# amazon-science/gnn-tail-generalization

Hardware: AMD Instinct MI355X
Metric: teachergnn_fullgraph_train_steps_per_sec (higher is better)
Workload: dtype f32

## Files before the change

### gnn-tail-generalization_amd/csrc/cb_front.hip

```cpp
#include "cb_common.h"
#include "cb_limb_core.h"
#include "cb_philox.h"
#include "cb_tile_gemm.h"

namespace cb {

struct FrontArgs {
  const float* x;
  int64_t ld_x;
  const uint4* image_in;
  const float* bias_in;
  const uint4* image_0;
  const float* rowscale;
  const float* addend;
  int64_t ld_add;
  float* x0;
  int64_t ld_x0;
  unsigned long long* bits;
  float* x0_drop;
  int64_t ld_drop;
  float* z0;
  int64_t ld_z;
  int64_t M;
  uint32_t thresh;
  float keep_scale;
  uint64_t seed_x, seed_x0;
  const uint64_t* seed_dev;
  int64_t row0;
  int n_tiles;
};

template <int NS1>
__global__ void __launch_bounds__(256, 2) k_front(FrontArgs fa) {
  constexpr int K1 = 16 * NS1, LDX = K1 + 4, NV = kTM * K1 / 4 / 256;
  static_assert(NV >= 1 && kTM * LDX <= kTM * kTLD, "x tile must fit the region of the X0 tile");
  __shared__ __attribute__((aligned(16))) float tile[kTM * kTLD];
  constexpr int kScratch = 2 * RowOperand<kTM>::BYTES > 4 * 8 * kCLD * 4 ? 2 * RowOperand<kTM>::BYTES : 4 * 8 * kCLD * 4;
  __shared__ __attribute__((aligned(16))) char scratch[kScratch];
  float (*cstrip)[8 * kCLD] = reinterpret_cast<float (*)[8 * kCLD]>(scratch);
  __shared__ float rs_tile[2][kTM];
  const int t = threadIdx.x, lane = t & 63, w = __builtin_amdgcn_readfirstlane(t >> 6);
  const uint64_t sx = fa.seed_dev ? fa.seed_x + *fa.seed_dev : fa.seed_x, s0 = fa.seed_dev ? fa.seed_x0 + *fa.seed_dev : fa.seed_x0;
  float4 xr[NV];
  auto load_x = [&](int tile_id) {
    const int64_t m0 = (int64_t)tile_id * kTM;
#pragma unroll
    for (int j = 0; j < NV; ++j) {
      const int idx = t + 256 * j, row = idx / (K1 / 4), c4 = idx % (K1 / 4);
      const int64_t m = m0 + row;
      xr[j] = (tile_id < fa.n_tiles && m < fa.M) ? *reinterpret_cast<const float4*>(fa.x + m * fa.ld_x + 4 * c4) : make_float4(0.f, 0.f, 0.f, 0.f);
    }
  };
  float bvec[4] = {0.f, 0.f, 0.f, 0.f};
  if (fa.bias_in) {
#pragma unroll
    for (int i = 0; i < 4; ++i) bvec[i] = fa.bias_in[4 * lane + i];
  }
  int par = 0;
  for (int tile_id = blockIdx.x; tile_id < fa.n_tiles; tile_id += gridDim.x, par ^= 1) {
    const int64_t m0 = (int64_t)tile_id * kTM;
    load_x(tile_id);
#pragma unroll
    for (int j = 0; j < NV; ++j) {
      const int idx = t + 256 * j, row = idx / (K1 / 4), c4 = idx % (K1 / 4);
      float v[4] = {xr[j].x, xr[j].y, xr[j].z, xr[j].w};
      if (fa.thresh) {
        float mk[4];
        keep4(sx, ((fa.row0 + m0 + row) * K1 + 4 * c4) >> 2, fa.thresh, fa.keep_scale, mk);
#pragma unroll
        for (int i = 0; i < 4; ++i) v[i] = mul_rounded(v[i], mk[i]);
      }
      *reinterpret_cast<float4*>(tile + row * LDX + 4 * c4) = make_float4(v[0], v[1], v[2], v[3]);
    }
    if (t < kTM) rs_tile[par][t] = (fa.rowscale && m0 + t < fa.M) ? fa.rowscale[m0 + t] : 1.f;
    __syncthreads();
    f32x16 acc[2][2];
    tile_times_image_coop<NS1, LDX, 1>(tile, scratch, fa.image_in, w, lane, t, acc);
    {
      const int l31 = lane & 31, lh = lane >> 5;
#pragma unroll
      for (int i = 0; i < 2; ++i)
#pragma unroll
        for (int j = 0; j < 2; ++j)
#pragma unroll
          for (int reg = 0; reg < 16; ++reg)
            tile[(32 * i + (reg & 3) + 8 * (reg >> 2) + 4 * lh) * kTLD + 64 * w + 32 * j + l31] = acc[i][j][reg];
    }
    __syncthreads();
#pragma unroll 4
    for (int r = 0; r < 16; ++r) {
      const int row = 16 * w + r;
      const int64_t m = m0 + row;
      float* tp = tile + row * kTLD + 4 * lane;
      const float4 v = *reinterpret_cast<const float4*>(tp);
      float o[4] = {v.x, v.y, v.z, v.w};
#pragma unroll
      for (int i = 0; i < 4; ++i) o[i] = fmaxf(o[i] + bvec[i], 0.f);
      float xd[4] = {o[0], o[1], o[2], o[3]};
      if (fa.thresh) {
        float mk[4];
        keep4(s0, ((fa.row0 + m) * kND + 4 * lane) >> 2, fa.thresh, fa.keep_scale, mk);
#pragma unroll
        for (int i = 0; i < 4; ++i) xd[i] = o[i] * mk[i];
      }
      *reinterpret_cast<float4*>(tp) = make_float4(xd[0], xd[1], xd[2], xd[3]);
      if (m < fa.M) {
        store_stream4(fa.x0 + m * fa.ld_x0 + 4 * lane, o);
        if (fa.bits) {
          unsigned long long mine = 0ull;
#pragma unroll
          for (int k = 0; k < 4; ++k) {
            const unsigned long long wq = __ballot(o[k] > 0.f);
            if (lane == k) mine = wq;
          }
          if (lane < 4) fa.bits[m * 4 + lane] = mine;
        }
        if (fa.x0_drop) store_stream4(fa.x0_drop + m * fa.ld_drop + 4 * lane, xd);
      }
    }
    __syncthreads();
    tile_times_image_coop<kNS, kTLD, 1>(tile, scratch, fa.image_0, w, lane, t, acc);
    acc_rows_through_strip(acc, cstrip[w], w, lane, [&](int row, int n, const float4& v) {
      const int64_t m = m0 + row;
      if (m < fa.M) {
        const float rs = rs_tile[par][row];
        float ad[4] = {0.f, 0.f, 0.f, 0.f};
        if (fa.addend) {
          const float4 a4 = *reinterpret_cast<const float4*>(fa.addend + m * fa.ld_add + n);
          ad[0] = a4.x; ad[1] = a4.y; ad[2] = a4.z; ad[3] = a4.w;
        }
        const float zero_bias = 0.f;
        float o[4] = {v.x, v.y, v.z, v.w};
#pragma unroll
        for (int e = 0; e < 4; ++e) o[e] = o[e] * rs + ad[e] + zero_bias;
        store_stream4(fa.z0 + m * fa.ld_z + n, o);
      }
    });
  }
}

static inline bool fr_al16(const void* p) { return ((uintptr_t)p % 16) == 0; }

}

using namespace cb;

extern "C" size_t cb_front_image_bytes(int64_t K) {
  if (K != 64 && K != 128) return 0;
  return (size_t)(K / 16) * kNT * 3 * 64 * sizeof(uint4);
}

extern "C" int cb_front_image_f32(const float* W, int64_t ld, int64_t K, int transpose, void* image, size_t image_bytes, void* stream) {
  CB_CHECK_ARG(cb_front_image_bytes(K) > 0, CB_E_INVALID, "cb_front_image_f32: K must be 64 or 128 (got %lld)", (long long)K);
  CB_CHECK_ARG(W && image && ld >= (transpose ? K : kND), CB_E_INVALID, "cb_front_image_f32: null pointer / bad leading dimension");
  CB_CHECK_ARG(image_bytes >= cb_front_image_bytes(K) && fr_al16(image), CB_E_WORKSPACE, "cb_front_image_f32: image buffer too small or misaligned");
  const int64_t sk = transpose ? 1 : ld, sn = transpose ? ld : 1;
  const int ns = (int)(K / 16);
  hipLaunchKernelGGL(k_weight_image, dim3(ns * kNT * 64 / 256), dim3(256), 0, (hipStream_t)stream, W, sk, sn, (uint4*)image, ns);
  CB_LAUNCH_CHECK();
  return CB_OK;
}

extern "C" int cb_trunk_front_f32(const float* x, int64_t ld_x, int64_t M, int64_t K, const void* image_in, const float* bias_in, const void* image_0,
                                  const float* rowscale, const float* addend, int64_t ld_add, float* x0, int64_t ld_x0, uint64_t* relu_bits,
                                  float* x0_drop, int64_t ld_drop, float* z0, int64_t ld_z, float drop_p, uint64_t seed_x, uint64_t seed_x0,
                                  const uint64_t* seed_dev, int64_t row0, void* stream) {
  CB_CHECK_ARG(M >= 0 && cb_front_image_bytes(K) > 0 && drop_p >= 0.f && drop_p < 1.f && row0 >= 0, CB_E_INVALID,
               "cb_trunk_front_f32: bad size (K must be 64 or 128; hidden width 256) or p");
  CB_CHECK_ARG(M < ((int64_t)1 << 31) * kTM / 2, CB_E_RANGE, "cb_trunk_front_f32: size out of range");
  if (M == 0) return CB_OK;
  CB_CHECK_ARG(x && image_in && image_0 && x0 && z0, CB_E_INVALID, "cb_trunk_front_f32: null pointer");
  CB_CHECK_ARG(fr_al16(x) && ld_x % 4 == 0 && ld_x >= K && fr_al16(image_in) && fr_al16(image_0) && fr_al16(x0) && ld_x0 % 4 == 0 && ld_x0 >= kND &&
                   fr_al16(z0) && ld_z % 4 == 0 && ld_z >= kND && (!addend || (fr_al16(addend) && ld_add % 4 == 0 && ld_add >= kND)) &&
                   (!x0_drop || (fr_al16(x0_drop) && ld_drop % 4 == 0 && ld_drop >= kND)) && (!relu_bits || (uintptr_t)relu_bits % 8 == 0),
               CB_E_INVALID, "cb_trunk_front_f32: 16-byte aligned rows required");
  FrontArgs fa{x, ld_x, (const uint4*)image_in, bias_in, (const uint4*)image_0, rowscale, addend, ld_add, x0, ld_x0, (unsigned long long*)relu_bits,
               x0_drop, ld_drop, z0, ld_z, M};
  fa.thresh = drop_p > 0.f ? dropout_threshold(drop_p) : 0u;
  fa.keep_scale = 1.f / (1.f - drop_p);
  fa.seed_x = seed_x; fa.seed_x0 = seed_x0; fa.seed_dev = seed_dev; fa.row0 = row0;
  fa.n_tiles = (int)((M + kTM - 1) / kTM);
  int dev = 0, n_cu = 0;
  if (hipGetDevice(&dev) != hipSuccess || hipDeviceGetAttribute(&n_cu, hipDeviceAttributeMultiprocessorCount, dev) != hipSuccess || n_cu <= 0) n_cu = 256;
  const int blocks = fa.n_tiles < 2 * n_cu ? fa.n_tiles : 2 * n_cu;
  const dim3 grid((unsigned)blocks), blk(256);
  hipStream_t st = (hipStream_t)stream;
  if (K == 64) hipLaunchKernelGGL((k_front<4>), grid, blk, 0, st, fa);
  else hipLaunchKernelGGL((k_front<8>), grid, blk, 0, st, fa);
  CB_LAUNCH_CHECK();
  return CB_OK;
}
```

### gnn-tail-generalization_amd/csrc/cb_tile_gemm.h

```cpp
#pragma once
#include "cb_common.h"
#include "cb_limb_core.h"

namespace cb {

constexpr int kTM = 64;
constexpr int kTLD = 260;
constexpr int kKD = 256;
constexpr int kND = 256;
constexpr int kNT = kND / 32, kNS = kKD / 16;

__global__ void __launch_bounds__(256) k_weight_image(const float* __restrict__ W, int64_t sk, int64_t sn, uint4* __restrict__ image, int n_steps);

__device__ __forceinline__ bf16x8 as_bf16x8(const uint4& v) { return __builtin_bit_cast(bf16x8, v); }

__device__ __forceinline__ void store_stream4(float* __restrict__ p, const float (&v)[4]) {
  typedef float f4_t __attribute__((ext_vector_type(4)));
  const f4_t q = {v[0], v[1], v[2], v[3]};
  __builtin_nontemporal_store(q, reinterpret_cast<f4_t*>(p));
}

template <int NSTEPS, int TLD, int PF = 1>
__device__ __forceinline__ void tile_times_image(const float* __restrict__ tile, const uint4* __restrict__ image, int w, int lane, f32x16 (&acc)[2][2]) {
  static_assert(PF >= 1 && PF <= 3 && PF < NSTEPS, "prefetch distance");
  const int l31 = lane & 31, lh = lane >> 5;
#pragma unroll
  for (int i = 0; i < 2; ++i)
#pragma unroll
    for (int j = 0; j < 2; ++j)
#pragma unroll
      for (int e = 0; e < 16; ++e) acc[i][j][e] = 0.f;
  const float* a_row[2] = {tile + l31 * TLD + 8 * lh, tile + (32 + l31) * TLD + 8 * lh};
  const uint4* bp = image + ((int64_t)(2 * w) * 3) * 64 + lane;
  uint4 bq[PF + 1][2][3];
#pragma unroll
  for (int d = 0; d < PF; ++d) {
#pragma unroll
    for (int j = 0; j < 2; ++j)
#pragma unroll
      for (int p = 0; p < 3; ++p) bq[d][j][p] = bp[j * 192 + p * 64];
    bp += kNT * 192;
  }
  auto step = [&](int s, int cur, int nx) {
    if (s + PF < NSTEPS) {
#pragma unroll
      for (int j = 0; j < 2; ++j)
#pragma unroll
        for (int p = 0; p < 3; ++p) bq[nx][j][p] = bp[j * 192 + p * 64];
    }
    bp += kNT * 192;
#pragma unroll
    for (int i = 0; i < 2; ++i) {
      const float4 x0 = *reinterpret_cast<const float4*>(a_row[i] + 16 * s);
      const float4 x1 = *reinterpret_cast<const float4*>(a_row[i] + 16 * s + 4);
      uint32_t hh[4], mm[4], ll[4];
      split3x2(x0.x, x0.y, hh[0], mm[0], ll[0]);
      split3x2(x0.z, x0.w, hh[1], mm[1], ll[1]);
      split3x2(x1.x, x1.y, hh[2], mm[2], ll[2]);
      split3x2(x1.z, x1.w, hh[3], mm[3], ll[3]);
      const bf16x8 a_hi = as_bf16x8(make_uint4(hh[0], hh[1], hh[2], hh[3]));
      const bf16x8 a_mid = as_bf16x8(make_uint4(mm[0], mm[1], mm[2], mm[3]));
      const bf16x8 a_lo = as_bf16x8(make_uint4(ll[0], ll[1], ll[2], ll[3]));
#define CB_TG_MFMA2(A_, P_) \
  _Pragma("unroll") for (int j = 0; j < 2; ++j) acc[i][j] = __builtin_amdgcn_mfma_f32_32x32x16_bf16(A_, as_bf16x8(bq[cur][j][P_]), acc[i][j], 0, 0, 0);
      CB_TG_MFMA2(a_lo, 0)
      CB_TG_MFMA2(a_hi, 2)
      CB_TG_MFMA2(a_mid, 1)
      CB_TG_MFMA2(a_mid, 0)
      CB_TG_MFMA2(a_hi, 1)
      CB_TG_MFMA2(a_hi, 0)
#undef CB_TG_MFMA2
    }
  };
  constexpr int R = PF + 1, MAIN = NSTEPS / R * R;
#pragma unroll 1
  for (int s0 = 0; s0 < MAIN; s0 += R) {
#pragma unroll
    for (int r = 0; r < R; ++r) step(s0 + r, r, (r + PF) % R);
  }
#pragma unroll
  for (int r = 0; r < NSTEPS - MAIN; ++r) step(MAIN + r, r, (r + PF) % R);
}

template <int NSTEPS, int TLD, int PF = 1>
__device__ __forceinline__ void tile_times_image_coop(const float* __restrict__ tile, char* __restrict__ planes, const uint4* __restrict__ image, int w, int lane,
                                                      int t, f32x16 (&acc)[2][2]) {
  using OA = RowOperand<kTM>;
  static_assert(OA::NV == 1 && PF >= 1 && PF <= 3 && PF < NSTEPS, "64-row tiles, one float4 of the slab per thread");
#pragma unroll
  for (int i = 0; i < 2; ++i)
#pragma unroll
    for (int j = 0; j < 2; ++j)
#pragma unroll
      for (int e = 0; e < 16; ++e) acc[i][j][e] = 0.f;
  const int row = t >> 2, kq = t & 3;
  const float* a_src = tile + row * TLD + 4 * kq;
  const uint32_t woff = row * 32 + (((kq >> 1) ^ ((row >> 3) & 1)) << 4) + ((kq & 1) << 3);
  const uint32_t aaddr[2] = {OA::frag_addr(0, lane), OA::frag_addr(32, lane)};
  auto stage = [&](int s, char* dst) {
    const float4 x = *reinterpret_cast<const float4*>(a_src + 16 * s);
    const float v[4] = {x.x, x.y, x.z, x.w};
    uint2 pl[3];
    split4(v, pl);
#pragma unroll
    for (int p = 0; p < 3; ++p) *reinterpret_cast<uint2*>(dst + p * OA::PLANE + woff) = pl[p];
  };
  const uint4* bp = image + ((int64_t)(2 * w) * 3) * 64 + lane;
  uint4 bq[PF + 1][2][3];
#pragma unroll
  for (int d = 0; d < PF; ++d) {
#pragma unroll
    for (int j = 0; j < 2; ++j)
#pragma unroll
      for (int p = 0; p < 3; ++p) bq[d][j][p] = bp[j * 192 + p * 64];
    bp += kNT * 192;
  }
  stage(0, planes);
  __syncthreads();
  auto step = [&](int s, int cur, int nx) {
    if (s + PF < NSTEPS) {
#pragma unroll
      for (int j = 0; j < 2; ++j)
#pragma unroll
        for (int p = 0; p < 3; ++p) bq[nx][j][p] = bp[j * 192 + p * 64];
    }
    bp += kNT * 192;
    const char* S = planes + (s & 1) * OA::BYTES;
    if (s + 1 < NSTEPS) stage(s + 1, planes + ((s + 1) & 1) * OA::BYTES);
#pragma unroll
    for (int i = 0; i < 2; ++i) {
      const bf16x8 a_lo = OA::frag(S, aaddr[i], 2), a_hi = OA::frag(S, aaddr[i], 0), a_mid = OA::frag(S, aaddr[i], 1);
#define CB_TG_MFMA2(A_, P_) \
  _Pragma("unroll") for (int j = 0; j < 2; ++j) acc[i][j] = __builtin_amdgcn_mfma_f32_32x32x16_bf16(A_, as_bf16x8(bq[cur][j][P_]), acc[i][j], 0, 0, 0);
      CB_TG_MFMA2(a_lo, 0)
      CB_TG_MFMA2(a_hi, 2)
      CB_TG_MFMA2(a_mid, 1)
      CB_TG_MFMA2(a_mid, 0)
      CB_TG_MFMA2(a_hi, 1)
      CB_TG_MFMA2(a_hi, 0)
#undef CB_TG_MFMA2
    }
    __syncthreads();
  };
  constexpr int R = PF + 1, MAIN = NSTEPS / R * R;
#pragma unroll 1
  for (int s0 = 0; s0 < MAIN; s0 += R) {
#pragma unroll
    for (int r = 0; r < R; ++r) step(s0 + r, r, (r + PF) % R);
  }
#pragma unroll
  for (int r = 0; r < NSTEPS - MAIN; ++r) step(MAIN + r, r, (r + PF) % R);
}

constexpr int kNTn = 2;
__global__ void __launch_bounds__(256) k_weight_image_narrow(const float* __restrict__ W, int64_t sk, int64_t sn, uint4* __restrict__ image, int n_steps,
                                                             int n_cols);

template <int NSTEPS, int TLD>
__device__ __forceinline__ void tile_times_image_block(const float* __restrict__ tile, const uint4* __restrict__ image, int i, int j, int lane, f32x16& acc) {
  const int l31 = lane & 31, lh = lane >> 5;
#pragma unroll
  for (int e = 0; e < 16; ++e) acc[e] = 0.f;
  const float* a_row = tile + (32 * i + l31) * TLD + 8 * lh;
  const uint4* bp = image + ((int64_t)j * 3) * 64 + lane;
  uint4 bq[2][3];
#pragma unroll
  for (int p = 0; p < 3; ++p) bq[0][p] = bp[p * 64];
  bp += kNTn * 192;
  auto step = [&](int s, int cur, int nx) {
    if (s + 1 < NSTEPS) {
#pragma unroll
      for (int p = 0; p < 3; ++p) bq[nx][p] = bp[p * 64];
    }
    bp += kNTn * 192;
    const float4 x0 = *reinterpret_cast<const float4*>(a_row + 16 * s);
    const float4 x1 = *reinterpret_cast<const float4*>(a_row + 16 * s + 4);
    uint32_t hh[4], mm[4], ll[4];
    split3x2(x0.x, x0.y, hh[0], mm[0], ll[0]);
    split3x2(x0.z, x0.w, hh[1], mm[1], ll[1]);
    split3x2(x1.x, x1.y, hh[2], mm[2], ll[2]);
    split3x2(x1.z, x1.w, hh[3], mm[3], ll[3]);
    const bf16x8 a_hi = as_bf16x8(make_uint4(hh[0], hh[1], hh[2], hh[3]));
    const bf16x8 a_mid = as_bf16x8(make_uint4(mm[0], mm[1], mm[2], mm[3]));
    const bf16x8 a_lo = as_bf16x8(make_uint4(ll[0], ll[1], ll[2], ll[3]));
    acc = __builtin_amdgcn_mfma_f32_32x32x16_bf16(a_lo, as_bf16x8(bq[cur][0]), acc, 0, 0, 0);
    acc = __builtin_amdgcn_mfma_f32_32x32x16_bf16(a_hi, as_bf16x8(bq[cur][2]), acc, 0, 0, 0);
    acc = __builtin_amdgcn_mfma_f32_32x32x16_bf16(a_mid, as_bf16x8(bq[cur][1]), acc, 0, 0, 0);
    acc = __builtin_amdgcn_mfma_f32_32x32x16_bf16(a_mid, as_bf16x8(bq[cur][0]), acc, 0, 0, 0);
    acc = __builtin_amdgcn_mfma_f32_32x32x16_bf16(a_hi, as_bf16x8(bq[cur][1]), acc, 0, 0, 0);
    acc = __builtin_amdgcn_mfma_f32_32x32x16_bf16(a_hi, as_bf16x8(bq[cur][0]), acc, 0, 0, 0);
  };
  static_assert(NSTEPS % 2 == 0, "K loop unrolled by two");
#pragma unroll 1
  for (int s0 = 0; s0 < NSTEPS; s0 += 2) {
    step(s0, 0, 1);
    step(s0 + 1, 1, 0);
  }
}

constexpr int kCLD = 68;

template <class F>
__device__ __forceinline__ void acc_rows_through_strip(const f32x16 (&acc)[2][2], float* __restrict__ cs, int w, int lane, F&& fn) {
  const int l31 = lane & 31, lh = lane >> 5;
#pragma unroll
  for (int i = 0; i < 2; ++i)
#pragma unroll
    for (int q = 0; q < 4; ++q) {
#pragma unroll
      for (int r4 = 0; r4 < 4; ++r4)
#pragma unroll
        for (int j = 0; j < 2; ++j) cs[(r4 + 4 * lh) * kCLD + 32 * j + l31] = acc[i][j][4 * q + r4];
#pragma unroll
      for (int half = 0; half < 2; ++half) {
        const int idx = lane + 64 * half, row = idx >> 4, c4 = (idx & 15) * 4;
        const float4 v = *reinterpret_cast<const float4*>(cs + row * kCLD + c4);
        fn(32 * i + 8 * q + row, 64 * w + c4, v);
      }
    }
}

}
```

Measured before the change: 9.242.

## Widen front kernel to 512 threads with one column block per wave

The fused front kernel moves from 256 threads (4 waves, each covering 64 output columns) to 512 threads (8 waves, each covering 32 columns). The shared tile-GEMM and strip-epilogue helpers are generalised over columns-per-wave and thread count, and only the first four waves stage the A operand. This halves accumulator registers per wave to allow more waves in flight and better latency hiding. In exchange, each wave's B-image load is amortised over fewer MFMAs, and the extra waves add barrier participation.

```diff
diff --git a/gnn-tail-generalization_amd/csrc/cb_front.hip b/gnn-tail-generalization_amd/csrc/cb_front.hip
--- a/gnn-tail-generalization_amd/csrc/cb_front.hip
+++ b/gnn-tail-generalization_amd/csrc/cb_front.hip
@@ -30,23 +30,30 @@
   int n_tiles;
 };
 
+constexpr int kFrontThreads = 512, kFrontWaves = kFrontThreads / 64;
+constexpr int kFrontWN = kNT / kFrontWaves;
+
 template <int NS1>
-__global__ void __launch_bounds__(256, 2) k_front(FrontArgs fa) {
-  constexpr int K1 = 16 * NS1, LDX = K1 + 4, NV = kTM * K1 / 4 / 256;
-  static_assert(NV >= 1 && kTM * LDX <= kTM * kTLD, "x tile must fit the region of the X0 tile");
+__global__ void __launch_bounds__(kFrontThreads, 4) k_front(FrontArgs fa) {
+  constexpr int K1 = 16 * NS1, LDX = K1 + 4, NV = kTM * K1 / 4 / kFrontThreads;
+  constexpr int RPW = kTM / kFrontWaves;
+  static_assert(NV >= 1 && kTM * K1 / 4 % kFrontThreads == 0 && kTM * LDX <= kTM * kTLD, "x tile must fit the region of the X0 tile");
   __shared__ __attribute__((aligned(16))) float tile[kTM * kTLD];
-  constexpr int kScratch = 2 * RowOperand<kTM>::BYTES > 4 * 8 * kCLD * 4 ? 2 * RowOperand<kTM>::BYTES : 4 * 8 * kCLD * 4;
+  constexpr int kStrip = 8 * strip_ld<kFrontWN>();
+  constexpr int kScratch = 2 * RowOperand<kTM>::BYTES > kFrontWaves * kStrip * 4 ? 2 * RowOperand<kTM>::BYTES : kFrontWaves * kStrip * 4;
   __shared__ __attribute__((aligned(16))) char scratch[kScratch];
-  float (*cstrip)[8 * kCLD] = reinterpret_cast<float (*)[8 * kCLD]>(scratch);
+  float (*cstrip)[kStrip] = reinterpret_cast<float (*)[kStrip]>(scratch);
   __shared__ float rs_tile[2][kTM];
   const int t = threadIdx.x, lane = t & 63, w = __builtin_amdgcn_readfirstlane(t >> 6);
   const uint64_t sx = fa.seed_dev ? fa.seed_x + *fa.seed_dev : fa.seed_x, s0 = fa.seed_dev ? fa.seed_x0 + *fa.seed_dev : fa.seed_x0;
   float4 xr[NV];
   auto load_x = [&](int tile_id) {
     const int64_t m0 = (int64_t)tile_id * kTM;
+    int tl = t;
+    asm volatile("" : "+v"(tl));
 #pragma unroll
     for (int j = 0; j < NV; ++j) {
-      const int idx = t + 256 * j, row = idx / (K1 / 4), c4 = idx % (K1 / 4);
+      const int idx = tl + kFrontThreads * j, row = idx / (K1 / 4), c4 = idx % (K1 / 4);
       const int64_t m = m0 + row;
       xr[j] = (tile_id < fa.n_tiles && m < fa.M) ? *reinterpret_cast<const float4*>(fa.x + m * fa.ld_x + 4 * c4) : make_float4(0.f, 0.f, 0.f, 0.f);
     }
@@ -60,9 +67,11 @@
   for (int tile_id = blockIdx.x; tile_id < fa.n_tiles; tile_id += gridDim.x, par ^= 1) {
     const int64_t m0 = (int64_t)tile_id * kTM;
     load_x(tile_id);
+    int tl = t;
+    asm volatile("" : "+v"(tl));
 #pragma unroll
     for (int j = 0; j < NV; ++j) {
-      const int idx = t + 256 * j, row = idx / (K1 / 4), c4 = idx % (K1 / 4);
+      const int idx = tl + kFrontThreads * j, row = idx / (K1 / 4), c4 = idx % (K1 / 4);
       float v[4] = {xr[j].x, xr[j].y, xr[j].z, xr[j].w};
       if (fa.thresh) {
         float mk[4];
@@ -74,22 +83,22 @@
     }
     if (t < kTM) rs_tile[par][t] = (fa.rowscale && m0 + t < fa.M) ? fa.rowscale[m0 + t] : 1.f;
     __syncthreads();
-    f32x16 acc[2][2];
-    tile_times_image_coop<NS1, LDX, 1>(tile, scratch, fa.image_in, w, lane, t, acc);
+    f32x16 acc[2][kFrontWN];
+    tile_times_image_coop<NS1, LDX, 1, kFrontWN, kFrontThreads>(tile, scratch, fa.image_in, w, lane, t, acc);
     {
       const int l31 = lane & 31, lh = lane >> 5;
 #pragma unroll
       for (int i = 0; i < 2; ++i)
 #pragma unroll
-        for (int j = 0; j < 2; ++j)
+        for (int j = 0; j < kFrontWN; ++j)
 #pragma unroll
           for (int reg = 0; reg < 16; ++reg)
-            tile[(32 * i + (reg & 3) + 8 * (reg >> 2) + 4 * lh) * kTLD + 64 * w + 32 * j + l31] = acc[i][j][reg];
+            tile[(32 * i + (reg & 3) + 8 * (reg >> 2) + 4 * lh) * kTLD + 32 * kFrontWN * w + 32 * j + l31] = acc[i][j][reg];
     }
     __syncthreads();
 #pragma unroll 4
-    for (int r = 0; r < 16; ++r) {
-      const int row = 16 * w + r;
+    for (int r = 0; r < RPW; ++r) {
+      const int row = RPW * w + r;
       const int64_t m = m0 + row;
       float* tp = tile + row * kTLD + 4 * lane;
       const float4 v = *reinterpret_cast<const float4*>(tp);
@@ -119,8 +128,8 @@
       }
     }
     __syncthreads();
-    tile_times_image_coop<kNS, kTLD, 1>(tile, scratch, fa.image_0, w, lane, t, acc);
-    acc_rows_through_strip(acc, cstrip[w], w, lane, [&](int row, int n, const float4& v) {
+    tile_times_image_coop<kNS, kTLD, 1, kFrontWN, kFrontThreads>(tile, scratch, fa.image_0, w, lane, t, acc);
+    acc_rows_through_strip<kFrontWN>(acc, cstrip[w], w, lane, [&](int row, int n, const float4& v) {
       const int64_t m = m0 + row;
       if (m < fa.M) {
         const float rs = rs_tile[par][row];
@@ -183,7 +192,7 @@
   int dev = 0, n_cu = 0;
   if (hipGetDevice(&dev) != hipSuccess || hipDeviceGetAttribute(&n_cu, hipDeviceAttributeMultiprocessorCount, dev) != hipSuccess || n_cu <= 0) n_cu = 256;
   const int blocks = fa.n_tiles < 2 * n_cu ? fa.n_tiles : 2 * n_cu;
-  const dim3 grid((unsigned)blocks), blk(256);
+  const dim3 grid((unsigned)blocks), blk(kFrontThreads);
   hipStream_t st = (hipStream_t)stream;
   if (K == 64) hipLaunchKernelGGL((k_front<4>), grid, blk, 0, st, fa);
   else hipLaunchKernelGGL((k_front<8>), grid, blk, 0, st, fa);
diff --git a/gnn-tail-generalization_amd/csrc/cb_tile_gemm.h b/gnn-tail-generalization_amd/csrc/cb_tile_gemm.h
--- a/gnn-tail-generalization_amd/csrc/cb_tile_gemm.h
+++ b/gnn-tail-generalization_amd/csrc/cb_tile_gemm.h
@@ -82,22 +82,25 @@
   for (int r = 0; r < NSTEPS - MAIN; ++r) step(MAIN + r, r, (r + PF) % R);
 }
 
-template <int NSTEPS, int TLD, int PF = 1>
+template <int NSTEPS, int TLD, int PF = 1, int WN = 2, int NTHR = 256>
 __device__ __forceinline__ void tile_times_image_coop(const float* __restrict__ tile, char* __restrict__ planes, const uint4* __restrict__ image, int w, int lane,
-                                                      int t, f32x16 (&acc)[2][2]) {
+                                                      int t, f32x16 (&acc)[2][WN]) {
   using OA = RowOperand<kTM>;
-  static_assert(OA::NV == 1 && PF >= 1 && PF <= 3 && PF < NSTEPS, "64-row tiles, one float4 of the slab per thread");
+  static_assert(OA::NV == 1 && PF >= 1 && PF <= 3 && PF < NSTEPS, "64-row tiles, one float4 of the slab per staging thread");
+  static_assert(NTHR % 256 == 0 && WN * (NTHR / 64) == kNT, "the block's wavefronts cover the 256 output columns");
 #pragma unroll
   for (int i = 0; i < 2; ++i)
 #pragma unroll
-    for (int j = 0; j < 2; ++j)
+    for (int j = 0; j < WN; ++j)
 #pragma unroll
       for (int e = 0; e < 16; ++e) acc[i][j][e] = 0.f;
-  const int row = t >> 2, kq = t & 3;
+  const bool stager = NTHR == 256 || w < 4;
+  const int row = (t & 255) >> 2, kq = t & 3;
   const float* a_src = tile + row * TLD + 4 * kq;
   const uint32_t woff = row * 32 + (((kq >> 1) ^ ((row >> 3) & 1)) << 4) + ((kq & 1) << 3);
   const uint32_t aaddr[2] = {OA::frag_addr(0, lane), OA::frag_addr(32, lane)};
   auto stage = [&](int s, char* dst) {
+    if (!stager) return;
     const float4 x = *reinterpret_cast<const float4*>(a_src + 16 * s);
     const float v[4] = {x.x, x.y, x.z, x.w};
     uint2 pl[3];
@@ -105,12 +108,12 @@
 #pragma unroll
     for (int p = 0; p < 3; ++p) *reinterpret_cast<uint2*>(dst + p * OA::PLANE + woff) = pl[p];
   };
-  const uint4* bp = image + ((int64_t)(2 * w) * 3) * 64 + lane;
-  uint4 bq[PF + 1][2][3];
+  const uint4* bp = image + ((int64_t)(WN * w) * 3) * 64 + lane;
+  uint4 bq[PF + 1][WN][3];
 #pragma unroll
   for (int d = 0; d < PF; ++d) {
 #pragma unroll
-    for (int j = 0; j < 2; ++j)
+    for (int j = 0; j < WN; ++j)
 #pragma unroll
       for (int p = 0; p < 3; ++p) bq[d][j][p] = bp[j * 192 + p * 64];
     bp += kNT * 192;
@@ -120,7 +123,7 @@
   auto step = [&](int s, int cur, int nx) {
     if (s + PF < NSTEPS) {
 #pragma unroll
-      for (int j = 0; j < 2; ++j)
+      for (int j = 0; j < WN; ++j)
 #pragma unroll
         for (int p = 0; p < 3; ++p) bq[nx][j][p] = bp[j * 192 + p * 64];
     }
@@ -131,7 +134,7 @@
     for (int i = 0; i < 2; ++i) {
       const bf16x8 a_lo = OA::frag(S, aaddr[i], 2), a_hi = OA::frag(S, aaddr[i], 0), a_mid = OA::frag(S, aaddr[i], 1);
 #define CB_TG_MFMA2(A_, P_) \
-  _Pragma("unroll") for (int j = 0; j < 2; ++j) acc[i][j] = __builtin_amdgcn_mfma_f32_32x32x16_bf16(A_, as_bf16x8(bq[cur][j][P_]), acc[i][j], 0, 0, 0);
+  _Pragma("unroll") for (int j = 0; j < WN; ++j) acc[i][j] = __builtin_amdgcn_mfma_f32_32x32x16_bf16(A_, as_bf16x8(bq[cur][j][P_]), acc[i][j], 0, 0, 0);
       CB_TG_MFMA2(a_lo, 0)
       CB_TG_MFMA2(a_hi, 2)
       CB_TG_MFMA2(a_mid, 1)
@@ -198,10 +201,13 @@
   }
 }
 
-constexpr int kCLD = 68;
-
-template <class F>
-__device__ __forceinline__ void acc_rows_through_strip(const f32x16 (&acc)[2][2], float* __restrict__ cs, int w, int lane, F&& fn) {
+template <int WN>
+constexpr int strip_ld() { return 32 * WN + 4; }
+constexpr int kCLD = strip_ld<2>();
+
+template <int WN = 2, class F>
+__device__ __forceinline__ void acc_rows_through_strip(const f32x16 (&acc)[2][WN], float* __restrict__ cs, int w, int lane, F&& fn) {
+  constexpr int CLD = strip_ld<WN>(), QPR = 8 * WN;
   const int l31 = lane & 31, lh = lane >> 5;
 #pragma unroll
   for (int i = 0; i < 2; ++i)
@@ -210,12 +216,12 @@
 #pragma unroll
       for (int r4 = 0; r4 < 4; ++r4)
 #pragma unroll
-        for (int j = 0; j < 2; ++j) cs[(r4 + 4 * lh) * kCLD + 32 * j + l31] = acc[i][j][4 * q + r4];
-#pragma unroll
-      for (int half = 0; half < 2; ++half) {
-        const int idx = lane + 64 * half, row = idx >> 4, c4 = (idx & 15) * 4;
-        const float4 v = *reinterpret_cast<const float4*>(cs + row * kCLD + c4);
-        fn(32 * i + 8 * q + row, 64 * w + c4, v);
+        for (int j = 0; j < WN; ++j) cs[(r4 + 4 * lh) * CLD + 32 * j + l31] = acc[i][j][4 * q + r4];
+#pragma unroll
+      for (int part = 0; part < WN; ++part) {
+        const int idx = lane + 64 * part, row = idx / QPR, c4 = (idx % QPR) * 4;
+        const float4 v = *reinterpret_cast<const float4*>(cs + row * CLD + c4);
+        fn(32 * i + 8 * q + row, 32 * WN * w + c4, v);
       }
     }
 }
```

New measurement: 9.297 (median of 6 runs). Within noise of the previous version (+0.6%).
